# pymlex/recommendation-system-pokec

Hardware: AMD Instinct MI355X
Metric: FAS candidates scored/sec over 1.6M users, top-k=10; 1/2/4/8 GPU + %HBM peak (higher is better)
Workload: dtype f64; 1 GPU; cfg2: full 1.6M-user single-query interest FAS all-candidates top-10; workload_key=cfg2_all_candidates_top10_1632803users_q1_shard1of1, topk=10, parallelism=candidate-shard x1, hw_queues=4

## Files before the change

recommendation-system-pokec_amd/csrc/pf_api.cpp:

```cpp
#include <hip/hip_runtime.h>

#include <algorithm>
#include <atomic>
#include <cmath>
#include <cstdlib>
#include <cstring>
#include <mutex>
#include <string>
#include <thread>
#include <unordered_map>
#include <unordered_set>
#include <vector>

#include "pf_batch.h"
#include "pf_ctx.h"
#include "pf_debug.h"
#include "pf_kernels.h"
#include "pf_store.h"
#include "pokec_fas.h"

using pf::DBuf;
using pf::PinBuf;
using pf::Ranked;
using pf::par_jobs;
// ... 178 lines not shown
        if (rc != PF_OK) return rc;
        g0 = g1;
    }
    return PF_OK;
}

int run_pairs(pf_ctx* c, const std::vector<int32_t>& qidx, const std::vector<std::vector<int32_t>>& slots,
              std::vector<std::vector<float>>& out, DBuf* keep = nullptr, std::vector<int64_t>* goff = nullptr,
              const pf::FieldSel& sel = pf::FieldSel{}, const pf::ProfileView* pv = nullptr) {
    out.assign(qidx.size(), {});
    if (keep) {
        size_t tot = 0;
        goff->assign(qidx.size(), 0);
        for (size_t g = 0; g < qidx.size(); ++g) {
            (*goff)[g] = (int64_t)tot;
            tot += slots[g].size();
        }
        HIPCHK(c, keep->ensure(std::max<size_t>(tot, 1) * sizeof(float)));
    }
    for (size_t g = 0; g < qidx.size(); ++g) out[g].assign(slots[g].size(), 0.f);
    return pair_chunks(c, qidx, slots, kPairThreads, (size_t)8u << 20, pv, [&](const PairChunk& k) -> int {
        HIPCHK(c, c->h_scores.ensure(k.npairs * sizeof(float)));
        float* dsc = nullptr;
        if (keep) {
            dsc = keep->as<float>() + (*goff)[k.g0];
        } else {
            HIPCHK(c, c->d_scores.ensure(k.npairs * sizeof(float)));
            dsc = c->d_scores.as<float>();
        }
        HIPCHK(c, pf::launch_pairs({.st = c->ds, .pool = c->d_pool.as<uint8_t>(), .refs_dev = c->d_refs.as<pf::QImageRef>(),
                                    .max_lds = k.im.max_lds, .gtab = k.im.gtab, .blocks = c->d_blocks.as<pf::PairBlock>(),
                                    .nblocks = k.nblocks, .order = nullptr, .slots = c->d_slots.as<int32_t>(),
                                    .out = dsc, .s = c->stream, .sel = sel}));
        c->jb.n_dispatch += k.nblocks != 0;
        const float* res = c->h_scores.as<float>();
        HIPCHK(c, hipMemcpyAsync(c->h_scores.p, dsc, k.npairs * sizeof(float), hipMemcpyDeviceToHost, c->stream));
        HIPCHK(c, hipStreamSynchronize(c->stream));
        k.hl.lap(pf::kHpGpu);
        par_jobs(k.g1 - k.g0, [&](size_t i) {
            const size_t g = k.g0 + i;
            if (!slots[g].empty()) std::memcpy(out[g].data(), res + k.gf[i], slots[g].size() * sizeof(float));
        }, 256);
        k.hl.lap(pf::kHpUnpack);
        return PF_OK;
    });
}

int run_pair_terms(pf_ctx* c, const std::vector<int32_t>& qidx, const std::vector<std::vector<int32_t>>& slots,
                   const std::vector<std::vector<int64_t>>& dest, pf_pair_terms_head* head, double* terms,
                   const pf::FieldSel& sel, const pf::ProfileView* pv = nullptr) {
    const size_t W = (size_t)(pf::kNumFixed + c->hc.T);
    const size_t max_pairs = ((size_t)256u << 20) / (W * sizeof(double));
    return pair_chunks(c, qidx, slots, (uint32_t)pf::kTermsPairs, max_pairs, pv, [&](const PairChunk& k) -> int {
        const size_t hb = k.npairs * sizeof(pf_pair_terms_head), tb = k.npairs * W * sizeof(double);
        HIPCHK(c, c->d_thead.ensure(hb));
        HIPCHK(c, c->d_terms.ensure(tb));
        HIPCHK(c, c->h_thead.ensure(hb));
        HIPCHK(c, c->h_terms.ensure(tb));
        HIPCHK(c, pf::launch_terms({.st = c->ds, .pool = c->d_pool.as<uint8_t>(), .refs_dev = c->d_refs.as<pf::QImageRef>(),
                                    .lds = (uint32_t)sizeof(pf::QConst) + k.im.max_img, .gtab = k.im.gtab,
                                    .blocks = c->d_blocks.as<pf::PairBlock>(), .nblocks = k.nblocks,
                                    .slots = c->d_slots.as<int32_t>(), .head = c->d_thead.as<pf_pair_terms_head>(),
                                    .terms = c->d_terms.as<double>(), .s = c->stream, .sel = sel}));
        HIPCHK(c, hipMemcpyAsync(c->h_thead.p, c->d_thead.p, hb, hipMemcpyDeviceToHost, c->stream));
        HIPCHK(c, hipMemcpyAsync(c->h_terms.p, c->d_terms.p, tb, hipMemcpyDeviceToHost, c->stream));
        HIPCHK(c, hipStreamSynchronize(c->stream));
        k.hl.lap(pf::kHpGpu);
        const pf_pair_terms_head* rh = c->h_thead.as<pf_pair_terms_head>();
        const double* rt = c->h_terms.as<double>();
        par_jobs(k.g1 - k.g0, [&](size_t i) {
            const size_t g = k.g0 + i;
            for (size_t j = 0; j < slots[g].size(); ++j) {
                head[dest[g][j]] = rh[k.gf[i] + j];
                std::memcpy(terms + (size_t)dest[g][j] * W, rt + (k.gf[i] + j) * W, W * sizeof(double));
            }
        }, 256);
        k.hl.lap(pf::kHpUnpack);
        return PF_OK;
    });
}

uint32_t post_mode(bool claimed) {
    static const long pr = pf::debug_long("k5_prune", 2);
    static const bool prs = pf::debug_long("k5_prune_stats", 0) != 0;
    const uint32_t p = pr <= 0 ? 0u : (pf::kPostPrune | (pr == 1 ? pf::kPostPruneBlockOnly : 0u) | (prs ? pf::kPostPruneStats : 0u));
    static const bool fko = pf::debug_long("k5_filter_blockout", 1) == 0;
    const uint32_t f = fko ? pf::kPostFiltKeepBlocks : 0u;
    return (claimed ? p : 0u) | f;
}

constexpr int kBatchBlocksPerWgDefault = 32;
int batch_blocks_per_wg() {
    static const int n = (int)std::max(1L, pf::debug_long("k5_batch_blocks", kBatchBlocksPerWgDefault));
    return n;
}

uint32_t post_image_lds(const pf::QPostHead* h) {
    return pf::post_lds(pf::post_var_lds(h->n_tok, h->n_tok + h->n_club + h->n_friend));
}
uint32_t filt_lds(const pf_ctx* c) { return c->filt.fields ? pf::kFiltLds : 0u; }

int scan_lanes();

int one_query_wgs(int resident, bool lanes) {
    static const long n = pf::debug_long("k5_wgs", 0);
    if (n > 0) return (int)n;
    if (!lanes) return resident;
    const int nl = scan_lanes();
    const int w = nl >= 12 ? resident * 3 / 16 : (nl >= 6 ? resident / 2 : (nl >= 3 ? resident * 7 / 8 : resident));
    return std::max(8, w & ~7);
}

int scan_events(pf_ctx* c, bool& timed, hipEvent_t& e0, hipEvent_t& e1) {
    e0 = c->ev0;
    e1 = c->ev1;
    const auto untimed = [&] {
        timed = false;
        c->last_ev0 = c->last_ev1 = nullptr;
        return (int)PF_OK;
    };
    if (!timed) return untimed();
    if (c->prof_on) {
        if (c->prof_seen++ % c->prof_every != 0) return untimed();
        if (c->prof_used == c->prof_ev.size()) {
            if (c->prof_ev.size() >= kProfCap) return untimed();
            hipEvent_t a, b;
            HIPCHK(c, pf::timing_event(&a));
            HIPCHK(c, pf::timing_event(&b));
            c->prof_ev.emplace_back(a, b);
        }
        e0 = c->prof_ev[c->prof_used].first;
        e1 = c->prof_ev[c->prof_used].second;
        ++c->prof_used;
    }
    return PF_OK;
}

struct LaneUse {
    pf_ctx::ScanLane* ln = nullptr;
    int row = 0;
    uint64_t* keys = nullptr;
};

int scan_lanes() {
    static const int n = (int)std::min((long)pf_ctx::kMaxLanes, pf::debug_long("scan_lanes", 3));
    return n;
}

int lane_begin(pf_ctx* c, hipStream_t caller, LaneUse& u) {
    u = LaneUse{};
    const int nlanes = scan_lanes();
    if (nlanes < 2 || caller == c->stream) return PF_OK;
    const int li = c->lane_cur;
    pf_ctx::ScanLane* ln = &c->lane[li];
    c->lane_cur = (li + 1) % nlanes;
    if (!ln->done) {
        HIPCHK(c, hipEventCreate(&ln->done));
        for (hipEvent_t& e : ln->freed) HIPCHK(c, hipEventCreateWithFlags(&e, hipEventDisableTiming));
    }
    const hipStream_t ls[3] = {c->stream, c->jb.aux, c->jb.aux2};
    ln->st = li < 3 ? ls[li] : c->lane_st[li];
    if (!ln->st) ln->st = c->stream;
    const int r = ln->row;
    ln->row = (r + 1) % pf_ctx::kLaneRows;
    const int g = r / pf_ctx::kLaneGroupRows;
    if (r % pf_ctx::kLaneGroupRows == 0 && ln->used[g]) HIPCHK(c, hipStreamWaitEvent(ln->st, ln->freed[g], 0));
    HIPCHK(c, ln->keys.ensure((size_t)pf_ctx::kLaneRows * pf::kMaxTopK * sizeof(uint64_t)));
    u.ln = ln;
    u.row = r;
    u.keys = ln->keys.as<uint64_t>() + (size_t)r * pf::kMaxTopK;
    return PF_OK;
// ... 1284 lines not shown
```

recommendation-system-pokec_amd/csrc/pf_kernels.hip:

```cpp
#include <hip/hip_ext.h>
#include <hip/hip_runtime.h>

#include <cstdint>
#include <algorithm>
#include <unordered_map>
#include <vector>
#include <cstdio>
#include <cstdlib>

#include "pf_device.h"
#include "pf_filter.h"
#include "pf_kernels.h"
#include "pf_plan.h"
#include "pf_prune.h"
#include "pf_select.h"

namespace pf {

static_assert(sizeof(QConst) % 16 == 0, "QConst must keep the LDS carve 16-B aligned");
static_assert(sizeof(QVal) == 16, "QVal is one 16-B load");

#ifdef PF_K5_TIMERS
__device__ unsigned long long g_k5t[16];
__device__ unsigned long long g_k1t[12];
// ... 859 lines not shown
}

__device__ __forceinline__ int set_list(const uint32_t* spre, int n, uint32_t f) {
    int lo = 0, hi = n - 1;
    while (lo < hi) {
        const int mid = (lo + hi + 1) >> 1;
        if (spre[mid] <= f) lo = mid; else hi = mid - 1;
    }
    return lo;
}

template <bool DEAD = false>
__device__ __forceinline__ void wave_prefix(uint32_t* gpre, const uint2* rng, int nl, int lane, const PTok* dead = nullptr) {
    uint32_t carry = 0;
    for (int b = 0; b < nl; b += 64) {
        const int j = b + lane;
        uint32_t len = j < nl ? rng[j].y - rng[j].x : 0u;
        if constexpr (DEAD) {
            if (j < nl && reinterpret_cast<const uint32_t*>(dead)[4 * j + 1] == kTokDeadHi) len = 0u;
        }
        uint32_t x = len;
        x = wave_incl_scan(x);
        if (j < nl) gpre[j] = carry + x - len;
        carry += wave_last(x);
    }
    if (lane == 0) gpre[nl] = carry;
}

__device__ __forceinline__ int round_list(const uint32_t* gpre, int ja, int jb, uint32_t g) {
    int j = ja;
#pragma unroll
    for (int s = 32; s > 0; s >>= 1) j += gpre[min(j + s, jb)] <= g ? s : 0;
    return j;
}

template <int CAP = kRoundCap>
__device__ __forceinline__ void build_map(uint64_t* mb, uint8_t* mc, uint2* mn, const uint32_t* gpre,
                                          const uint2* rng, int ja, int jb, int lane) {
    constexpr int kMW = CAP / 64;
    const uint32_t g0 = gpre[ja];
    const int j = ja + lane;
    uint32_t s = 0;
    bool ne = false;
    if (j < jb) {
        s = gpre[j] - g0;
        ne = gpre[j + 1] - g0 > s && s < (uint32_t)CAP;
    }
    if (lane < kMW) mb[lane] = 0ull;
    const uint64_t bal = __ballot(ne);
    const uint32_t k = (uint32_t)__popcll(bal & low_bits((uint32_t)lane));
    wave_sync();
    if (ne) {
        atomicOr(reinterpret_cast<unsigned long long*>(&mb[s >> 6]), 1ull << (s & 63u));
        mn[k] = make_uint2(rng[j].x - s, (uint32_t)lane);
    }
    wave_sync();
    const uint32_t c = lane < kMW ? (uint32_t)__popcll(mb[lane]) : 0u, x = wave_incl_scan(c);
    if (lane < kMW) mc[lane] = (uint8_t)(x - c);
}

constexpr uint32_t kItemRunShift = 11, kItemSlotMask = (1u << kItemRunShift) - 1u, kItemRunMax = 31;
static_assert(kRoundCap <= (int)kItemSlotMask + 1, "item slots fit 11 bits");
__device__ __forceinline__ uint32_t hit_run(uint64_t m, uint32_t lo, uint32_t hi) {
    return min((uint32_t)__popcll((m >> lo) & low_bits(hi - lo)), kItemRunMax);
}
__device__ __forceinline__ double run_dot(const double* slot, uint32_t r, uint32_t run, double dot) {
    for (uint32_t k = 1; k < run; k += 4) {
        double v[4];
#pragma unroll
        for (int u = 0; u < 4; ++u) v[u] = k + u < run ? slot[r + k + u] : 0.0;
#pragma unroll
        for (int u = 0; u < 4; ++u)
            if (k + u < run) dot += v[u];
    }
    return dot;
}

__device__ __forceinline__ double tok_product(const PTok* pt, int j, uint32_t tf) {
    const PTok v = pt[j];
    return v.wq * ((double)tf * v.idf);
}


__device__ __forceinline__ bool prune_record(ScanSync* sy, uint64_t best, int k, uint32_t c0, uint32_t c1,
                                             uint32_t thb, int lane) {
    uint32_t sb = 0u;
    bool rec = false;
    if (lane < k && best != ~0ull) {
        const uint32_t idx = (uint32_t)best ^ 0x80000000u;
        sb = __float_as_uint(key_score(best));
        rec = idx >= c0 && idx <= c1 && sb >= thb && prune_bin(sb) >= 0;
    }
    const uint64_t bal = __ballot(rec);
    if (bal == 0ull) return false;
    if (lane == __ffsll((unsigned long long)bal) - 1)
        __hip_atomic_fetch_add(&sy->hist[prune_bin(sb)], 1u, __ATOMIC_RELAXED, __HIP_MEMORY_SCOPE_AGENT);
    return true;
}

static __device__ __attribute__((noinline)) uint32_t prune_derive(ScanSync* sy, int k, uint32_t thb, int lane) {
    constexpr int kPer = (kPruneBins + 63) / 64;
    uint32_t cb[kPer], s = 0u;
#pragma unroll
    for (int i = 0; i < kPer; ++i) {
        const int b = kPruneBins - 1 - (kPer * lane + i);
        cb[i] = b >= 0 ? __hip_atomic_load(&sy->hist[b], __ATOMIC_RELAXED, __HIP_MEMORY_SCOPE_AGENT) : 0u;
        s += cb[i];
    }
    const uint32_t incl = wave_incl_scan(s);
    uint32_t run = incl - s, nt = 0u;
    if (run < (uint32_t)k && incl >= (uint32_t)k) {
        int bin = 0;
        bool got = false;
#pragma unroll
        for (int i = 0; i < kPer; ++i) {
            run += cb[i];
            if (!got && run >= (uint32_t)k) {
                got = true;
                bin = kPruneBins - 1 - (kPer * lane + i);
            }
        }
        nt = prune_edge(bin);
        if (nt > thb) __hip_atomic_fetch_max(&sy->theta, nt, __ATOMIC_RELAXED, __HIP_MEMORY_SCOPE_AGENT);
    }
    nt = wave_max_u32(nt);
    return nt > thb ? nt : thb;
}

#ifdef PF_K5_TIMERS
#define K5T(slot) do { const uint64_t t_ = clock64(); tacc[slot] += t_ - tprev; tprev = t_; } while (0)
#else
#define K5T(slot) do { } while (0)
#endif

#ifndef PF_K5_MINB
#define PF_K5_MINB 4
#endif
template <bool XD, bool FILT, bool SEL>
__global__ __launch_bounds__(kPostThreads, PF_K5_MINB) void fas_post_kernel(PostStore ps, const uint8_t* __restrict__ pool,
                                                              const uint32_t* __restrict__ img_off, int32_t blk_begin,
                                                              int32_t blk_end, int32_t k, uint64_t* __restrict__ parts,
                                                              ScanSync* __restrict__ sync, uint64_t* __restrict__ out,
                                                              const int32_t* __restrict__ out_rows, uint32_t mode,
                                                              const uint8_t* __restrict__ qconst, CandFilter F,
                                                              FieldSel S) {
    extern __shared__ __attribute__((aligned(16))) char smem[];
    const int qy = XD ? 0 : (int)blockIdx.y;
    const int bx = (int)blockIdx.x;
    const int nbx = (int)gridDim.x;
    const uint8_t* img = pool + img_off[qy];
    const uint8_t* qcp = qconst ? qconst : img;
    QPostHead H = *reinterpret_cast<const QPostHead*>(img + sizeof(QConst));
    const QTok* toks = reinterpret_cast<const QTok*>(img + H.tok_off);
    const QCol* cols = reinterpret_cast<const QCol*>(img + H.col_off);
    const PList* sets = reinterpret_cast<const PList*>(img + H.set_off);
    const int n_act_img = H.n_act;
    if constexpr (SEL) {
        if (!(S.fixed & kSelClubs)) { sets += H.n_club; H.n_club = 0; }
        if (!(S.fixed & kSelFriends)) H.n_friend = 0;
        int na = 0;
        for (int j = 0; j < n_act_img; ++j) na += (int)((S.cols >> cols[j].t) & 1ull);
        H.n_act = na;
    }
    const uint32_t* excl = reinterpret_cast<const uint32_t*>(img + H.excl_off);
    const int tid = (int)threadIdx.x, lane = tid & 63;
    char* base = smem + sizeof(QConst);
    uint64_t* mask = reinterpret_cast<uint64_t*>(base + kLdsMask);
    double* slot = reinterpret_cast<double*>(base + kLdsSlot);
    uint16_t* hit = reinterpret_cast<uint16_t*>(base + kLdsHit);
    uint16_t* hbase = reinterpret_cast<uint16_t*>(base + kLdsHbase);
    uint16_t* item = reinterpret_cast<uint16_t*>(base + kLdsItem);
    uint32_t* cnt = reinterpret_cast<uint32_t*>(base + kLdsCnt);
    uint32_t* exb = reinterpret_cast<uint32_t*>(base + kLdsExb);
    uint32_t* misc = reinterpret_cast<uint32_t*>(base + kLdsMisc);
    QCol* scol = reinterpret_cast<QCol*>(base + kLdsCols);
    double* ftab = reinterpret_cast<double*>(base + kLdsFtab);
    uint32_t* seg = reinterpret_cast<uint32_t*>(base + kLdsSeg);
    const int nsets = H.n_club + H.n_friend;
    const int nl = H.n_tok + nsets;
    PTok* pt = reinterpret_cast<PTok*>(base + kPostFixedLds);
    uint2* rng = reinterpret_cast<uint2*>(pt + H.n_tok);
    uint2* rtab = rng + nl;
    uint32_t* gpre = reinterpret_cast<uint32_t*>(rtab + H.n_tok + 1);
    uint32_t* spre = gpre + H.n_tok + 1;
    uint8_t* colof = reinterpret_cast<uint8_t*>(spre + nsets + 1);
    uint64_t* mapb = reinterpret_cast<uint64_t*>(base + kLdsMapB);
    uint2* mapn = reinterpret_cast<uint2*>(base + kLdsMapN);
    uint8_t* mapc = reinterpret_cast<uint8_t*>(base + kLdsMapC);
    uint64_t* lmk = reinterpret_cast<uint64_t*>(base + kLdsLmk);
    uint64_t* cpre = reinterpret_cast<uint64_t*>(base + kLdsCpre);
    double* need = reinterpret_cast<double*>(base + kLdsNeed);
    const bool prune = XD && (mode & kPostPrune) != 0u;
    const bool prune_rnd = prune && !(mode & kPostPruneBlockOnly);
    const bool pstats = XD && (mode & kPostPruneStats) != 0u;
    const bool drop = FILT || prune;
    CandFilter* fl = reinterpret_cast<CandFilter*>(
        smem + (((uint32_t)(reinterpret_cast<char*>(colof) + H.n_tok - smem) + 15u) & ~15u));
    if constexpr (FILT) {
        if (tid == 0) *fl = F;
    }
    if (tid < 16) misc[tid] = 0u;
    stage(smem, qcp, sizeof(QConst));
    if constexpr (!SEL) {
        for (int j = tid; j < H.n_act; j += kPostThreads) {
            const QCol c = cols[j];
            scol[j] = c;
            for (int x = c.j0; x < c.j1; ++x) colof[x] = (uint8_t)j;
        }
        if (tid == 0) {
            uint64_t m = 0;
            for (int j = 0; j < H.n_act; ++j) { cpre[j] = m; m |= 1ull << cols[j].t; }
            cpre[H.n_act] = m;
        }
        for (int j = tid; j <= kNumFixed + kPostMaxCols; j += kPostThreads)
            ftab[j] = (double)j / (double)(kNumFixed + reinterpret_cast<const QConst*>(qcp)->n_cols);
    } else {
        for (int j = tid; j < n_act_img; j += kPostThreads) {
            const QCol c = cols[j];
            int js = 0;
            for (int x = 0; x < j; ++x) js += (int)((S.cols >> cols[x].t) & 1ull);
            const bool on = (S.cols >> c.t) & 1ull;
            if (on) scol[js] = c;
            for (int x = c.j0; x < c.j1; ++x) colof[x] = on ? (uint8_t)js : kColDead;
        }
        if (tid == 0) {
            uint64_t m = 0;
            int js = 0;
            for (int j = 0; j < n_act_img; ++j) {
                const int t = cols[j].t;
                if ((S.cols >> t) & 1ull) { cpre[js++] = m; m |= 1ull << t; }
            }
            cpre[js] = m;
        }
        const int ncs = select_ncols(S.cols, reinterpret_cast<const QConst*>(qcp)->n_cols);
        for (int j = tid; j <= kNumFixed + kPostMaxCols; j += kPostThreads)
            ftab[j] = (double)j / (double)(kNumFixed + ncs);
        __syncthreads();
        if (tid == 0) select_apply(*reinterpret_cast<QConst*>(smem), S);
    }
    for (int j = tid; j < H.n_tok; j += kPostThreads) {
        const QTok t = toks[j];
        pt[j] = PTok{t.wq, t.idf};
        if constexpr (SEL) {
            if (colof[j] == kColDead) reinterpret_cast<uint32_t*>(pt + j)[1] = kTokDeadHi;
        }
    }
    __syncthreads();
    const QConst& q = *reinterpret_cast<const QConst*>(smem);
    uint64_t best = ~0ull;
#ifdef PF_K5_TIMERS
    uint64_t tacc[14] = {0};
    uint64_t tprev = clock64();
    const uint64_t tstart = tprev;
#endif
    const uint32_t B = (uint32_t)ps.bsize;
    const uint32_t cend = min((uint32_t)blk_end * B, (uint32_t)ps.n);
    const bool short_excl = H.n_excl <= kPostThreads;
    const uint32_t ex0 = short_excl && H.n_excl > 0 ? excl[min(tid, H.n_excl - 1)] : ~0u;
    const int pb = (nbx & 7) == 0 ? (bx & 7) * (nbx >> 3) + (bx >> 3) : bx;
    const int xng = min(8, nbx), xg = bx % xng;
    const int x_lo = blk_begin + (int)((int64_t)(blk_end - blk_begin) * xg / xng);
    const int x_hi = blk_begin + (int)((int64_t)(blk_end - blk_begin) * (xg + 1) / xng);
    const int x_nwg = (nbx - xg + xng - 1) / xng;
    unsigned int* xctr = &sync[qy].xcd_next[xg * 16];
    const int blk_last = XD ? x_hi : blk_end;
    for (int blk = XD ? x_lo + bx / xng : blk_begin + pb; blk < blk_last;) {
        unsigned int xclaim = 0;
        auto next_block = [&](bool now) __attribute__((always_inline)) {
            if constexpr (XD) {
                if (tid == 0) misc[0] = (uint32_t)(x_lo + x_nwg) + (now ? atomicAdd(xctr, 1u) : xclaim);
                __syncthreads();
                blk = (int)misc[0];
            } else {
                __syncthreads();
                blk += nbx;
            }
        };
        const uint32_t c0 = (uint32_t)blk * B;
        const uint32_t c1 = min(c0 + B, cend) - 1;
#ifdef PF_K5_BLOCKLOG
        const unsigned long long blog_t0 = __builtin_amdgcn_s_memrealtime();
#endif
        uint4 ha[kCandsPerThread], hb[kCandsPerThread];
#pragma unroll
        for (int kk = 0; kk < kCandsPerThread; ++kk) {
            const uint32_t c = min(c0 + kk * kPostThreads + tid, c1);
            ha[kk] = ps.hdr[2 * (size_t)c];
            hb[kk] = ps.hdr[2 * (size_t)c + 1];
        }
        uint32_t thb = 0u;
        if (prune) thb = __hip_atomic_load(&sync[qy].theta, __ATOMIC_RELAXED, __HIP_MEMORY_SCOPE_AGENT);
#pragma unroll 1
        for (int j = tid; j < nl; j += kPostThreads)
            rng[j] = list_range(ps, j < H.n_tok ? toks[j].l : sets[j - H.n_tok], c0, c1);
#pragma unroll
        for (int kk = 0; kk < kCandsPerThread; ++kk) {
            const uint32_t c = c0 + kk * kPostThreads + tid;
            if (!(c <= c1 && (uint32_t)(kk * kPostThreads + tid) < B)) {
                ha[kk] = make_uint4(0, 0, 0, 0);
                hb[kk] = make_uint4(0, 0, 0, 0);
            }
            cnt[kk * kPostThreads + tid] = 0u;
            mask[kk * kPostThreads + tid] = 0ull;
        }
        if (tid < kBlockCands / 32) exb[tid] = 0u;
        K5T(0);
        if constexpr (FILT) {
            uint32_t fskip = 0;
            bool any = false;
            const CandFilter f = *fl;
#pragma unroll
            for (int kk = 0; kk < kCandsPerThread; ++kk) {
                const bool there = c0 + kk * kPostThreads + tid <= c1 && (uint32_t)(kk * kPostThreads + tid) < B;
                const bool ok = filter_pass_post(f, ha[kk], hb[kk]);
                if (there && !ok) fskip |= 1u << kk;
                any |= there && ok;
            }
            if (!__syncthreads_or(any) && !(mode & kPostFiltKeepBlocks)) {
                if (pstats && tid == 0) {
                    misc[8] += c1 - c0 + 1u;
                    misc[11] += 1u;
                    misc[12] += thb == 0u ? 1u : 0u;
                }
                next_block(true);
                continue;
            }
#pragma unroll
            for (int kk = 0; kk < kCandsPerThread; ++kk) {
                const uint64_t bal = __ballot((fskip >> kk) & 1u);
                const uint32_t w = (uint32_t)(bal >> (lane & 32));
                if ((lane & 31) == 0 && w != 0u) atomicOr(&exb[(kk * kPostThreads + tid) >> 5], w);
            }
        } else {
            __syncthreads();
        }
        K5T(1);
        if (prune && tid >= kPostThreads - 64) {
            thb = (uint32_t)__builtin_amdgcn_readfirstlane((int)thb);
            if (misc[5] != 0u) {
                thb = prune_derive(sync + qy, k, thb, lane);
                wave_sync();
                if (lane == 0) misc[5] = 0u;
            }
            const int u = tid - (kPostThreads - 64);
            if (u == 0) misc[4] = thb;
            if (u >= 0 && u <= kNumFixed + kPostMaxCols) need[u] = prune_need(thb, u, kNumFixed + q.n_cols);
        }
        if (tid < 64) {
            ColPlan cpl = col_tokens(scol, H.n_act, lane);
            wave_prefix<SEL>(gpre, rng, H.n_tok, lane, pt);
            wave_sync();
            col_ends(cpl, gpre, H.n_act, lane);
            {
                int ci0 = 0, j0 = 0, nr = 0;
                while (ci0 < H.n_act) {
                    if constexpr (SEL) j0 = max(j0, __builtin_amdgcn_readlane(cpl.j0, ci0));
                    const Round Rr = plan_round(cpl, gpre, H.n_act, lane, ci0, j0);
                    if (lane == 0)
                        rtab[nr] = make_uint2((uint32_t)Rr.ja | (uint32_t)Rr.jb << 16, (uint32_t)Rr.ca | (uint32_t)Rr.ce << 16);
                    if (nr == 0) build_map(mapb, mapc, mapn, gpre, rng, Rr.ja, Rr.jb, lane);
                    ++nr;
                }
                if (lane == 0) misc[3] = (uint32_t)nr;
            }
        }
        if (short_excl) {
            const uint32_t p = ex0 - c0;
            if (tid < H.n_excl && p < B) atomicOr(&exb[p >> 5], 1u << (p & 31));
        } else {
            uint32_t lo = 0, hi = (uint32_t)H.n_excl;
            while (lo < hi) {
                const uint32_t mid = (lo + hi) >> 1;
                if (excl[mid] < c0) lo = mid + 1; else hi = mid;
            }
            hi = (uint32_t)H.n_excl;
            for (uint32_t b = lo; b < hi; b += kPostThreads) {
                const uint32_t x = b + tid;
                const uint32_t e = x < hi ? excl[x] : ~0u;
                const uint32_t p = e - c0;
                if (p < B) atomicOr(&exb[p >> 5], 1u << (p & 31));
                if (__syncthreads_or(e >= c0 + B)) break;
            }
        }
        if (tid >= 64 && nsets > 0) {
            wave_prefix(spre, rng + H.n_tok, nsets, lane);
            wave_sync();
            const uint32_t tot = spre[nsets];
            constexpr uint32_t kSetThreads = kPostThreads - 64;
            for (uint32_t f0 = (uint32_t)tid - 64u; f0 < tot; f0 += 2u * kSetThreads) {
                int js[2];
                uint32_t e[2];
#pragma unroll
                for (int u = 0; u < 2; ++u) {
                    const uint32_t f = f0 + u * kSetThreads;
                    js[u] = f < tot ? set_list(spre, nsets, f) : -1;
                    e[u] = js[u] >= 0 ? ps.post[K5CHK(rng[H.n_tok + js[u]].x + (f - spre[js[u]]), ps.n_post, 3)] : 0u;
                }
#pragma unroll
                for (int u = 0; u < 2; ++u) {
                    const uint32_t p = (e[u] >> 8) - c0;
                    if (js[u] >= 0 && p < B) atomicAdd(&cnt[p], (e[u] & 0xFFu) << (js[u] < H.n_club ? 0 : 16));
                }
            }
        }
        K5T(2);
        __syncthreads();
        K5T(1);
        double sum[kCandsPerThread];
        uint32_t used = 0;
        uint64_t pend[kCandsPerThread];
        uint32_t skip = 0;
#pragma unroll
        for (int kk = 0; kk < kCandsPerThread; ++kk) {
            const int p = kk * kPostThreads + tid;
            const uint32_t ct = cnt[p];
            if ((uint32_t)p >= B || c0 + p > c1 || ((exb[p >> 5] >> (p & 31)) & 1u)) skip |= 1u << kk;
            const uint64_t cm = (uint64_t)ha[kk].x | ((uint64_t)(ha[kk].y & 0xFFFFu) << 32);
            pend[kk] = cm & q.colmask;
            double s = 0.0;
            int u = 0;
            header_terms(q, (ha[kk].y >> 16) & 0xFFu, ha[kk].y >> 24, (int)(int16_t)(ha[kk].z & 0xFFFFu),
                         (int)(int16_t)(ha[kk].z >> 16), (int)hb[kk].x, (int)hb[kk].y, (int)hb[kk].z, s, u);
            set_terms(q, (int)(ct & 0xFFFFu), ha[kk].w & 0xFFFFu, (int)(ct >> 16), ha[kk].w >> 16, s, u);
// ... 212 lines not shown
                if (cf.j0 < ja) t_in = cf.t;
                if (cl.j1 > jb) t_on = cl.t;
            }
#pragma unroll
            for (int kk = 0; kk < kCandsPerThread; ++kk) {
                const int p = kk * kPostThreads + tid;
                uint64_t mr = F > 0 ? mask[p] : 0ull;
                uint32_t rr = F > 0 ? hbase[p] : 0u;
                for (uint64_t pr = pend[kk] & rtm; pr; pr &= pr - 1) {
                    const int t = __ffsll((unsigned long long)pr) - 1;
                    const uint64_t lm = lmk[t];
                    const uint64_t h = mr & lm;
                    mr &= ~lm;
                    const uint32_t r0 = rr;
                    rr += (uint32_t)__popcll(h);
                    if (t != t_in && t != t_on) {
                        sum[kk] += h ? slot[r0] : q.sig0_col[t];
                        continue;
                    }
                    if (h) {
                        uint64_t v = h;
                        uint32_t r = r0;
                        while (v) {
                            const int jr = __ffsll((unsigned long long)v) - 1;
                            v &= v - 1;
                            cdot[kk] += tok_product(pt, ja + jr, hit[r++] & 0xFFu);
                        }
                        cnrm[kk] = slot[r0];
                        chit |= 1u << kk;
                    }
                    if (t != t_on) {
                        const bool hh = (chit >> kk) & 1u;
                        sum[kk] += (hh && cdot[kk] != 0.0) ? text_term(q, t, cdot[kk], cnrm[kk]) : q.sig0_col[t];
                        cdot[kk] = 0.0;
                        chit &= ~(1u << kk);
                    }
                }
                if (F > 0) mask[p] = 0ull;
            }
            if (prune_rnd && rnd + 1 < nrounds) {
                const uint64_t togo = ~(cpre[R.ce] & ~(t_on >= 0 ? 1ull << t_on : 0ull));
#pragma unroll
                for (int kk = 0; kk < kCandsPerThread; ++kk) {
                    const bool d = !((skip >> kk) & 1u) &&
                                   prune_dead(sum[kk], (double)__popcll(pend[kk] & togo), need[(used >> (8 * kk)) & 0xFFu]);
                    if (d) {
                        skip |= 1u << kk;
                        pend[kk] = 0ull;
                    }
                    if (pstats) {
                        const uint64_t bal = __ballot(d);
                        if (lane == 0) atomicAdd(&misc[10], (uint32_t)__popcll(bal));
                    }
                }
            }
            K5T(10);
            if (F == 0 && rnd + 1 < nrounds) {
                if (tid < 64) {
                    const uint2 r1 = rtab[rnd + 1];
                    const int nb = mbuf ^ 1;
                    build_map(mapb + nb * kMapWords, mapc + nb * kMapWords, mapn + nb * kRoundToks, gpre, rng,
                              (int)(r1.x & 0xFFFFu), (int)(r1.x >> 16), lane);
                }
                __syncthreads();
            }
            if (F > 0) __syncthreads();
        }
        K5T(11);
        uint64_t keys[kCandsPerThread];
#pragma unroll
        for (int kk = 0; kk < kCandsPerThread; ++kk) {
            uint64_t key = ~0ull;
            if (!((skip >> kk) & 1u)) {
                const int uk = (int)((used >> (8 * kk)) & 0xFFu);
                const float f = fas_score(sum[kk], uk, ftab[uk]);
                key = score_key(f, (int32_t)(c0 + kk * kPostThreads + tid));
            }
            keys[kk] = key;
        }
        static_assert(kCandsPerThread == 2, "2-key sort");
        if (keys[1] < keys[0]) { const uint64_t x = keys[0]; keys[0] = keys[1]; keys[1] = x; }
#pragma unroll
        for (int kk = 0; kk < kCandsPerThread; ++kk) topk_push(best, keys[kk], k, lane);
        if (prune && prune_record(sync + qy, best, k, c0, c1, misc[4], lane) && lane == 0) misc[5] = 1u;
        K5T(12);
#ifdef PF_K5_BLOCKLOG
        if (tid == 0) {
            const unsigned i = atomicAdd(&g_blog_n, 1u);
            if (i < kBlogCap) {
                g_blog_t[2 * i] = blog_t0;
                g_blog_t[2 * i + 1] = __builtin_amdgcn_s_memrealtime();
                g_blog_meta[i] = (unsigned)bx | (unsigned)blk << 16;
            }
        }
#endif
        next_block(false);
    }
#ifdef PF_K5_TIMERS
    tacc[13] = clock64() - tstart;
    if (lane == 0) {
        for (int i = 0; i < 14; ++i) atomicAdd(&g_k5t[i], (unsigned long long)tacc[i]);
        atomicAdd(&g_k5t[15], 1ull);
    }
#endif
    if (pstats) {
        __syncthreads();
        if (tid < kPruneStats) atomicAdd(&g_k5_prune[tid], (unsigned long long)misc[8 + tid]);
    }
    if (lane < k && best != ~0ull) {
        const uint32_t idx = (uint32_t)best ^ 0x80000000u;
        best = (best & 0xFFFFFFFF00000000ull) | (ps.hdr[2 * (size_t)idx + 1].w ^ 0x80000000u);
    }
    uint64_t* sc = reinterpret_cast<uint64_t*>(slot);

    post_tail(best, k, sc, sync, parts, out, out_rows, qy, bx, nbx);
}

constexpr int kMergeThreads = 1024;
__global__ __launch_bounds__(kMergeThreads) void topk_merge_kernel(const uint64_t* __restrict__ in, int32_t nparts,
                                                                   int64_t part_stride, int64_t query_stride, int32_t k,
                                                                   uint64_t* __restrict__ out,
                                                                   const int32_t* __restrict__ out_rows) {
    __shared__ uint64_t sc[16 * 64];
    const int q = blockIdx.x, lane = threadIdx.x & 63, wave = threadIdx.x >> 6;
    const int64_t total = (int64_t)nparts * k;
    uint64_t list = ~0ull;
    for (int64_t base = 0; base < total; base += (int64_t)blockDim.x * 8) {
        uint64_t x[8];
#pragma unroll
        for (int u = 0; u < 8; ++u) {
            const int64_t i = base + (int64_t)u * blockDim.x + threadIdx.x;
            x[u] = ~0ull;
            if (i < total) {
                const int32_t part = (int32_t)(i / k), j = (int32_t)(i - (int64_t)part * k);
                x[u] = in[(int64_t)part * part_stride + q * query_stride + j];
            }
        }
#pragma unroll
        for (int u = 0; u < 8; ++u) topk_push(list, x[u], k, lane);
    }
    if (lane < k) sc[wave * k + lane] = list;
    __syncthreads();
    if (wave == 0) {
        uint64_t acc = ~0ull;
        const int n = (int)(blockDim.x >> 6) * k;
        for (int b = 0; b < n; b += 64) topk_push(acc, b + lane < n ? sc[b + lane] : ~0ull, k, lane);
        const int row = out_rows ? out_rows[q] : q;
        if (lane < k) out[(size_t)row * k + lane] = acc;
    }
}

#ifdef PF_K1P_WPE
#define PF_K1P_BOUNDS __launch_bounds__(kPairThreads) __attribute__((amdgpu_waves_per_eu(PF_K1P_WPE, PF_K1P_WPE)))
#else
#define PF_K1P_BOUNDS __launch_bounds__(kPairThreads, 4)
#endif
template <bool PACKED, bool GTAB>
__global__ PF_K1P_BOUNDS void fas_pairs_kernel(DevStore st, const uint8_t* __restrict__ pool,
                                                        const QImageRef* __restrict__ refs,
                                                        const PairBlock* __restrict__ blocks,
                                                        const int32_t* __restrict__ order,
                                                        const int32_t* __restrict__ slots, float* __restrict__ out,
                                                        FieldSel S) {
    extern __shared__ __attribute__((aligned(16))) char smem[];
#ifdef PF_K5_TIMERS
    const uint64_t t0 = clock64();
    uint64_t tw[4] = {0, 0, 0, 0};
    uint64_t* twp = tw;
#else
    uint64_t* twp = nullptr;
#endif
    const PairBlock b = blocks[order ? order[blockIdx.x] : (int)blockIdx.x];
    const int i = (int)threadIdx.x;
    int p = i < b.count ? slots[b.begin + i] : -1;
    const bool active = p >= 0;
    if (!__syncthreads_or(active)) return;
    const PairHdr H = load_pair_hdr(st, p, active);
    char* scratch;
    const QView v = stage_query<GTAB>(smem, pool, refs[b.qimg], &scratch, S);
// ... 252 lines not shown
```

recommendation-system-pokec_amd/csrc/pf_prune.h:

```cpp
#pragma once
#include <stdint.h>

#if defined(__HIPCC__)
#define PF_HD __host__ __device__
#else
#define PF_HD
#endif

namespace pf {

constexpr uint32_t kPruneShift = 15;
constexpr uint32_t kPruneLowBits = 0x3E000000u;
constexpr uint32_t kPruneOneBits = 0x3F800000u;
constexpr int kPruneBase = (int)(kPruneLowBits >> kPruneShift);
constexpr int kPruneBins = (int)(kPruneOneBits >> kPruneShift) - kPruneBase + 1;

PF_HD inline int prune_bin(uint32_t bits) {
    if (bits < kPruneLowBits || bits >= 0x80000000u) return -1;
    const uint32_t b = bits >> kPruneShift, top = kPruneOneBits >> kPruneShift;
    return (int)(b < top ? b : top) - kPruneBase;
}
PF_HD inline uint32_t prune_edge(int bin) { return (uint32_t)(bin + kPruneBase) << kPruneShift; }

PF_HD inline float prune_float(uint32_t bits) {
    union { uint32_t u; float f; } v;
    v.u = bits;
    return v.f;
}

PF_HD inline double prune_need(uint32_t theta_bits, int u, int nterms) {
    if (theta_bits == 0u) return 0.0;
    const double t = (double)prune_float(theta_bits) * (1.0 - 1.0 / 1048576.0);
    const double F = (double)u / (double)nterms;
    const double d = 2.0 * F - t;
    if (!(d > 0.0)) return __builtin_huge_val();
    return (double)u * (t * F) / d;
}

PF_HD inline bool prune_dead(double acc, double remaining, double need) { return acc + remaining + 1e-9 < need; }

}
```

Measured before the change: 15.10 billion candidates/s.

## Defer prune histogram atomics and enable pruning for batched queries

```diff
diff --git a/recommendation-system-pokec_amd/csrc/pf_api.cpp b/recommendation-system-pokec_amd/csrc/pf_api.cpp
--- a/recommendation-system-pokec_amd/csrc/pf_api.cpp
+++ b/recommendation-system-pokec_amd/csrc/pf_api.cpp
@@ -284,11 +284,12 @@
 
 uint32_t post_mode(bool claimed) {
     static const long pr = pf::debug_long("k5_prune", 2);
+    static const bool prb = pf::debug_long("k5_prune_batch", 1) != 0;
     static const bool prs = pf::debug_long("k5_prune_stats", 0) != 0;
     const uint32_t p = pr <= 0 ? 0u : (pf::kPostPrune | (pr == 1 ? pf::kPostPruneBlockOnly : 0u) | (prs ? pf::kPostPruneStats : 0u));
     static const bool fko = pf::debug_long("k5_filter_blockout", 1) == 0;
     const uint32_t f = fko ? pf::kPostFiltKeepBlocks : 0u;
-    return (claimed ? p : 0u) | f;
+    return ((claimed || prb) ? p : 0u) | f;
 }
 
 constexpr int kBatchBlocksPerWgDefault = 32;
diff --git a/recommendation-system-pokec_amd/csrc/pf_kernels.hip b/recommendation-system-pokec_amd/csrc/pf_kernels.hip
--- a/recommendation-system-pokec_amd/csrc/pf_kernels.hip
+++ b/recommendation-system-pokec_amd/csrc/pf_kernels.hip
@@ -965,8 +965,8 @@
 }
 
 
-__device__ __forceinline__ bool prune_record(ScanSync* sy, uint64_t best, int k, uint32_t c0, uint32_t c1,
-                                             uint32_t thb, int lane) {
+__device__ __forceinline__ void prune_fold(uint32_t* word, uint64_t best, int k, uint32_t c0, uint32_t c1,
+                                           uint32_t thb, int lane) {
     uint32_t sb = 0u;
     bool rec = false;
     if (lane < k && best != ~0ull) {
@@ -975,38 +975,41 @@
         rec = idx >= c0 && idx <= c1 && sb >= thb && prune_bin(sb) >= 0;
     }
     const uint64_t bal = __ballot(rec);
-    if (bal == 0ull) return false;
-    if (lane == __ffsll((unsigned long long)bal) - 1)
-        __hip_atomic_fetch_add(&sy->hist[prune_bin(sb)], 1u, __ATOMIC_RELAXED, __HIP_MEMORY_SCOPE_AGENT);
-    return true;
-}
-
-static __device__ __attribute__((noinline)) uint32_t prune_derive(ScanSync* sy, int k, uint32_t thb, int lane) {
-    constexpr int kPer = (kPruneBins + 63) / 64;
-    uint32_t cb[kPer], s = 0u;
-#pragma unroll
-    for (int i = 0; i < kPer; ++i) {
-        const int b = kPruneBins - 1 - (kPer * lane + i);
-        cb[i] = b >= 0 ? __hip_atomic_load(&sy->hist[b], __ATOMIC_RELAXED, __HIP_MEMORY_SCOPE_AGENT) : 0u;
-        s += cb[i];
-    }
-    const uint32_t incl = wave_incl_scan(s);
-    uint32_t run = incl - s, nt = 0u;
-    if (run < (uint32_t)k && incl >= (uint32_t)k) {
-        int bin = 0;
-        bool got = false;
-#pragma unroll
-        for (int i = 0; i < kPer; ++i) {
-            run += cb[i];
-            if (!got && run >= (uint32_t)k) {
-                got = true;
-                bin = kPruneBins - 1 - (kPer * lane + i);
-            }
-        }
-        nt = prune_edge(bin);
-        if (nt > thb) __hip_atomic_fetch_max(&sy->theta, nt, __ATOMIC_RELAXED, __HIP_MEMORY_SCOPE_AGENT);
+    if (bal == 0ull) return;
+    if (lane == __ffsll((unsigned long long)bal) - 1) atomicMax(word, sb);
+}
+
+static_assert(kMaxTopK < (1 << kPruneShift), "k rides in a theta's low bits");
+static __device__ __attribute__((noinline)) uint32_t prune_derive(ScanSync* sy, uint32_t thk, uint32_t rec) {
+    constexpr uint32_t kLow = (1u << kPruneShift) - 1u;
+    const int lane = (int)(threadIdx.x & 63u), k = (int)(thk & kLow);
+    const uint32_t thb = thk & ~kLow;
+    const int ns = prune_slabs(thb), rb = prune_bin(rec);
+    uint32_t cb[kPruneSlabs];
+#pragma unroll
+    for (int i = 0; i < kPruneSlabs; ++i) {
+        const int b = prune_slab_bin(i, lane);
+        cb[i] = 0u;
+        if (i < ns && prune_bin_live(b, thb)) cb[i] = __hip_atomic_load(&sy->hist[b], __ATOMIC_RELAXED, __HIP_MEMORY_SCOPE_AGENT);
+    }
+    const uint32_t cur = __hip_atomic_load(&sy->theta, __ATOMIC_RELAXED, __HIP_MEMORY_SCOPE_AGENT);
+    uint32_t above = 0u, nt = 0u;
+#pragma unroll
+    for (int i = 0; i < kPruneSlabs; ++i) {
+        if (i < ns && above < (uint32_t)k) {
+            const int b = prune_slab_bin(i, lane);
+            const uint32_t c = cb[i] + ((b == rb && prune_bin_live(b, thb)) ? 1u : 0u);
+            const uint32_t incl = wave_incl_scan(c);
+            if (prune_pick(above, incl, c, (uint32_t)k)) nt = prune_edge(b);
+            above += wave_last(incl);
+        }
     }
     nt = wave_max_u32(nt);
+    if (lane == 0) {
+        __hip_atomic_fetch_add(&sy->hist[rb], 1u, __ATOMIC_RELAXED, __HIP_MEMORY_SCOPE_AGENT);
+        if (nt > thb && nt > cur) __hip_atomic_fetch_max(&sy->theta, nt, __ATOMIC_RELAXED, __HIP_MEMORY_SCOPE_AGENT);
+    }
+    nt = nt > cur ? nt : cur;
     return nt > thb ? nt : thb;
 }
 
@@ -1073,9 +1076,9 @@
     uint64_t* lmk = reinterpret_cast<uint64_t*>(base + kLdsLmk);
     uint64_t* cpre = reinterpret_cast<uint64_t*>(base + kLdsCpre);
     double* need = reinterpret_cast<double*>(base + kLdsNeed);
-    const bool prune = XD && (mode & kPostPrune) != 0u;
+    const bool prune = (mode & kPostPrune) != 0u;
     const bool prune_rnd = prune && !(mode & kPostPruneBlockOnly);
-    const bool pstats = XD && (mode & kPostPruneStats) != 0u;
+    const bool pstats = (mode & kPostPruneStats) != 0u;
     const bool drop = FILT || prune;
     CandFilter* fl = reinterpret_cast<CandFilter*>(
         smem + (((uint32_t)(reinterpret_cast<char*>(colof) + H.n_tok - smem) + 15u) & ~15u));
@@ -1220,8 +1223,9 @@
         K5T(1);
         if (prune && tid >= kPostThreads - 64) {
             thb = (uint32_t)__builtin_amdgcn_readfirstlane((int)thb);
-            if (misc[5] != 0u) {
-                thb = prune_derive(sync + qy, k, thb, lane);
+            const uint32_t rec = misc[5];
+            if (rec != 0u) {
+                thb = prune_derive(sync + qy, thb | (uint32_t)k, rec);
                 wave_sync();
                 if (lane == 0) misc[5] = 0u;
             }
@@ -1600,7 +1604,7 @@
         if (keys[1] < keys[0]) { const uint64_t x = keys[0]; keys[0] = keys[1]; keys[1] = x; }
 #pragma unroll
         for (int kk = 0; kk < kCandsPerThread; ++kk) topk_push(best, keys[kk], k, lane);
-        if (prune && prune_record(sync + qy, best, k, c0, c1, misc[4], lane) && lane == 0) misc[5] = 1u;
+        if (prune) prune_fold(&misc[5], best, k, c0, c1, misc[4], lane);
         K5T(12);
 #ifdef PF_K5_BLOCKLOG
         if (tid == 0) {
@@ -1613,6 +1617,13 @@
         }
 #endif
         next_block(false);
+    }
+    if (prune && tid == kPostThreads - 64) {
+        const uint32_t rec = misc[5];
+        if (rec != 0u) {
+            const uint32_t old = __hip_atomic_fetch_add(&sync[qy].hist[prune_bin(rec)], 1u, __ATOMIC_RELAXED, __HIP_MEMORY_SCOPE_AGENT);
+            asm volatile("" ::"v"(old));
+        }
     }
 #ifdef PF_K5_TIMERS
     tacc[13] = clock64() - tstart;
diff --git a/recommendation-system-pokec_amd/csrc/pf_prune.h b/recommendation-system-pokec_amd/csrc/pf_prune.h
--- a/recommendation-system-pokec_amd/csrc/pf_prune.h
+++ b/recommendation-system-pokec_amd/csrc/pf_prune.h
@@ -28,6 +28,15 @@
     return v.f;
 }
 
+constexpr int kPruneSlab = 64;
+constexpr int kPruneSlabs = (kPruneBins + kPruneSlab - 1) / kPruneSlab;
+PF_HD inline int prune_slab_bin(int slab, int lane) { return kPruneBins - 1 - (kPruneSlab * slab + lane); }
+PF_HD inline bool prune_bin_live(int bin, uint32_t thb) { return bin > prune_bin(thb); }
+PF_HD inline int prune_slabs(uint32_t thb) { return (kPruneBins - 1 - prune_bin(thb) + kPruneSlab - 1) / kPruneSlab; }
+PF_HD inline bool prune_pick(uint32_t above, uint32_t incl, uint32_t c, uint32_t k) {
+    return above + incl >= k && above + incl - c < k;
+}
+
 PF_HD inline double prune_need(uint32_t theta_bits, int u, int nterms) {
     if (theta_bits == 0u) return 0.0;
     const double t = (double)prune_float(theta_bits) * (1.0 - 1.0 / 1048576.0);
```

Measured after the change: 17.12 billion candidates/s (median of 6 runs). 13.4% higher.
